# cure-lab/PnPInversion

Hardware: AMD Instinct MI355X
Metric: edited images/sec @ 512x512, 50 DDIM-inv + 50 denoise steps (higher is better)
Workload: dtype f16 (fp32 accumulate; latents / scheduler math fp32); 1 GPU; single 512x512 image per rank, SD-1.x (seeded synthetic weights), directinversion+p2p, faithful schedule: 650 UNet sample-forwards + 1 VAE encode + 5 VAE decodes per image, Refine+Reweight+LocalBlend controller; text K/V projected once per loop (not per forward); ddim_steps=50, schedule=lockstep

## Files before the change

### pnpinversion_amd/csrc/api.hip

```cpp
#include <math.h>
#include <stdio.h>
#include <stdlib.h>
#include <string.h>

#include <algorithm>
#include <functional>
#include <memory>
#include <string>

#include "model.h"

static int g_text_kv = 1;
static int g_temb_cache = 1;

static int fail(pnpi_ctx* c, int status, const char* what) {
  c->err = what;
  return status;
}
static int fail_launch(pnpi_ctx* c, int code, const char* what) {
  char buf[640];
  if (code > 0) {
    snprintf(buf, sizeof(buf), "HIP error %d (%s) in %s", code, hipGetErrorString((hipError_t)code), what);
    c->err = buf;
    return PNPI_EHIP;
// ... 201 lines not shown
  void* arena = nullptr;
  if (c->warena_ref && c->warena_ref->refs.fetch_sub(1) == 1) { arena = c->warena_ref->base; delete c->warena_ref; }
  void* bufs[] = {arena, c->persist.base, c->temp.base, c->ctrl_arena.base, c->splitk_ws, c->gn_partial, c->gn_bwd_ws,
                  c->temb_table, c->temb_h, c->temb_emb, c->bias_scratch, c->bias_tab, c->tkv.base, c->rows_ident};
  for (void* b : bufs) (void)hipFree(b);
  if (c->tape) {
    (void)hipFree(c->tape->garena.base); (void)hipFree(c->tape->d_ctx); (void)hipFree(c->tape->attn_scratch);
    for (auto& kv : c->tape->wd) (void)hipFree(kv.second);
    delete c->tape;
  }
  delete c;
}

static void invalidate_derived(pnpi_ctx* c) {
  std::fill(c->bias_valid.begin(), c->bias_valid.end(), 0);
  c->tkv.rows = 0; c->tkv.use = false;
  if (c->tape) { for (auto& kv : c->tape->wd) (void)hipFree(kv.second); c->tape->wd.clear(); }
}

int pnpi_load_weights(pnpi_ctx* c, const pnpi_named_tensor* ts, int n) {
  if (!c || !ts) return PNPI_EINVAL;
  if (c->warena_borrowed) return fail(c, PNPI_ESTATE, "this context borrows its weights (pnpi_create_shared): load them into the owning context");
  invalidate_derived(c);
  for (int i = 0; i < n; ++i) {
    const pnpi_named_tensor& t = ts[i];
    std::string name = t.name;
    size_t pos = name.find(".downsamplers.0.Conv2d_0.");
    if (pos != std::string::npos) name.replace(pos, strlen(".downsamplers.0.Conv2d_0."), ".downsamplers.0.conv.");
    if (name.compare(0, 16, "clip.text_model.") == 0) name = "clip." + name.substr(16);
    auto it = c->slots.find(name);
    if (it == c->slots.end()) continue;
    Slot& s = it->second;
    size_t numel = 1;
    for (int d = 0; d < t.ndim; ++d) numel *= (size_t)t.shape[d];
    if (s.kind == 0) {
      if (numel != (size_t)s.rows * s.cols * s.taps) { c->err = "shape mismatch for " + name; return PNPI_ESHAPE; }
      CK(launch_repack_matrix(t.data, t.dtype, s.rows, s.cols, s.taps, (half_t*)s.dst, s.dst_ld, s.cin_pad, s.row0, s.dh, s.Dp, c->st,
                              s.ilv_half));
    } else {
      if (numel != (size_t)s.n) { c->err = "shape mismatch for " + name; return PNPI_ESHAPE; }
      CK(launch_repack_vec(t.data, t.dtype, s.n, (float*)s.dst, c->st, s.ilv_half));
    }
    s.loaded = true;
  }
  return 0;
}

int pnpi_missing_weights(const pnpi_ctx* c, char* names_out, size_t cap) {
  int missing = 0;
  size_t used = 0;
  if (names_out && cap) names_out[0] = 0;
  for (auto& kv : c->slots)
    if (!kv.second.loaded && kv.first.compare(0, 5, "clip.") != 0) {
      ++missing;
      if (names_out && used + kv.first.size() + 2 < cap) {
        memcpy(names_out + used, kv.first.c_str(), kv.first.size());
        used += kv.first.size();
        names_out[used++] = '\n';
        names_out[used] = 0;
      }
    }
  return missing;
}

int pnpi_weight_arena(pnpi_ctx* c, void** ptr, size_t* bytes) {
  if (!c || !ptr || !bytes) return PNPI_EINVAL;
  *ptr = c->warena.base; *bytes = c->warena.cap;
  return 0;
}

int pnpi_mark_all_loaded(pnpi_ctx* c) {
  invalidate_derived(c);
  for (auto& kv : c->slots) kv.second.loaded = true;
  return 0;
}

int pnpi_set_scheduler(pnpi_ctx* c, const float* ac, int n_train, float final_alpha) {
  if (!c || !ac || n_train != c->cfg.n_train_timesteps) return PNPI_EINVAL;
  c->ac.assign(ac, ac + n_train);
  c->final_alpha = final_alpha;
  c->sched_set = true;
  return 0;
}

int pnpi_get_counters(const pnpi_ctx* c, pnpi_counters* out) { if (!c || !out) return PNPI_EINVAL; *out = c->ctr; return 0; }
int pnpi_reset_counters(pnpi_ctx* c) { if (!c) return PNPI_EINVAL; memset(&c->ctr, 0, sizeof(c->ctr)); return 0; }

__global__ void __launch_bounds__(512, 2) mfma_clock_kernel(int iters, float* sink) {
  const int lane = threadIdx.x & 63;
  unsigned h = (unsigned)(blockIdx.x * 512 + threadIdx.x) * 2654435761u;
  half8 a, b;
#pragma unroll
  for (int j = 0; j < 8; ++j) {
    h ^= h >> 16; h *= 0x85ebca6bu; h ^= h >> 13;
    a[j] = (half_t)((float)(h & 0xffff) * (2.f / 65536.f) - 1.f);
    b[j] = (half_t)((float)(h >> 16) * (2.f / 65536.f) - 1.f);
// ... 322 lines not shown
int pnpi_op_conv(pnpi_ctx* c, const void* x1, const void* x2, int C1, int C2, int B, int H, int W, int ksize, int stride, int pad,
                 int ups, int Ho, int Wo, const void* w, const float* bias, const void* res, int N, void* out, int force_cfg,
                 int force_split) {
  return conv_hook(c, x1, x2, C1, C2, B, H, W, ksize, stride, pad, ups, Ho, Wo, w, bias, res, N, out, force_cfg, force_split, nullptr, nullptr);
}
int pnpi_op_conv_stats(pnpi_ctx* c, const void* x1, const void* x2, int C1, int C2, int B, int H, int W, int ksize, int stride, int pad,
                       int ups, int Ho, int Wo, const void* w, const float* bias, const void* res, int N, void* out, int force_cfg,
                       int force_split, float* stats_out, int* tile_rows_out) {
  if (!c || !stats_out || !tile_rows_out) return PNPI_EINVAL;
  return conv_hook(c, x1, x2, C1, C2, B, H, W, ksize, stride, pad, ups, Ho, Wo, w, bias, res, N, out, force_cfg, force_split, stats_out, tile_rows_out);
}
int pnpi_tile_table_lookup(int M, int N, int K, int ksize, int* cfg, int* split, int* entry_m) {
  return igemm_table_lookup(M, N, K, ksize, cfg, split, entry_m);
}
int pnpi_set_tuning(const char* key, int value) {
  if (!key) return PNPI_EINVAL;
  if (!strcmp(key, "text_kv")) { g_text_kv = value; return 0; }
  if (!strcmp(key, "temb_cache")) { g_temb_cache = value; return 0; }
  if (!strcmp(key, "gn_inline_rows")) { norm_set_tuning_gn_inline_rows(value); return 0; }
  if (!strcmp(key, "attn_vt_perm")) { g_vt_perm = value; return 0; }
  if (!strcmp(key, "attn_aug")) { g_attn_aug = value; return 0; }
  if (!strcmp(key, "attn_pipe")) return attn_set_tuning_pipe(value) == 0 ? 0 : PNPI_EINVAL;
  if (!strcmp(key, "gn_slab")) { g_gn_slab = value; return 0; }
  if (!strcmp(key, "op_attention_aug")) { g_op_attention_aug = value; return 0; }
  if (!strcmp(key, "op_attention_vt_perm")) { g_op_attention_vt_perm = value; return 0; }
  if (!strcmp(key, "attn_bwd_flash")) { g_attn_bwd_flash = value; return 0; }
  return igemm_set_tuning(key, value) == 0 ? 0 : PNPI_EINVAL;
}
int pnpi_op_gemm(pnpi_ctx* c, const void* a, int lda, const void* w, int ldw, int M, int N, int K, float alpha, const float* bias,
                 const void* res, void* out, int ldo, int vt_col0, void* outT, int vt_ld, int vt_f32, int rpb, int force_cfg,
                 int force_split) {
  GemmP p; gemm_defaults(p);
  p.x1 = (const half_t*)a; p.C1 = K; p.ldx1 = lda; p.B = 1; p.H = 1; p.W = M; p.Ho = 1; p.Wo = M; p.ksize = 1;
  p.w = (const half_t*)w; p.ldw = ldw; p.M = M; p.N = N; p.K = K; p.alpha = alpha; p.bias = bias; p.res = (const half_t*)res;
  p.ldres = N; p.out = (half_t*)out; p.ldo = ldo;
  if (outT) { p.outT = outT; p.vt_col0 = vt_col0; p.vt_ld = vt_ld; p.vt_f32 = vt_f32; p.rows_per_batch = rpb; }
  CK(launch_igemm(p, c->splitk_ws, c->splitk_bytes, c->st, force_cfg, force_split));
  return 0;
}
int pnpi_op_gemm_geglu(pnpi_ctx* c, const void* a, int lda, const void* w, int ldw, int M, int N, int K, const float* bias, void* out,
                       int ldo) {
  GemmP p; gemm_defaults(p);
  p.x1 = (const half_t*)a; p.C1 = K; p.ldx1 = lda; p.B = 1; p.H = 1; p.W = M; p.Ho = 1; p.Wo = M; p.ksize = 1;
  p.w = (const half_t*)w; p.ldw = ldw; p.M = M; p.N = N; p.K = K; p.bias = bias; p.out = (half_t*)out; p.ldo = ldo; p.geglu = 1;
  CK(launch_igemm(p, c->splitk_ws, c->splitk_bytes, c->st));
  return 0;
// ... 112 lines not shown
```

### pnpinversion_amd/csrc/api_graph.inc

```
static void prof_open(pnpi_ctx* c, ProfRec& r) {
  (void)hipEventCreate(&r.a); (void)hipEventCreate(&r.b);
  (void)hipEventRecord(r.a, c->st);
}
static void prof_close(pnpi_ctx* c, ProfRec& r, int cls, double flops, double bytes, int M = 0, int N = 0, int K = 0, int ks = 0) {
  (void)hipEventRecord(r.b, c->st);
  r.cls = cls; r.flops = flops; r.bytes = bytes; r.M = M; r.N = N; r.K = K; r.ksize = ks;
  c->prof.push_back(r);
}
static int g_gn_slab = 0;
static int flush_pending(pnpi_ctx* c) {
  if (!c->pend_on) return 0;
  c->pend_on = false;
  return launch_splitk_reduce(c->pend, c->st);
}
#define PROF(cls, flops, bytes, expr) PROFD(cls, flops, bytes, 0, 0, 0, expr)
#define PROFD(cls, flops, bytes, d0, d1, d2, expr)            \
  do {                                                        \
    if (c->pend_on) { int _f = flush_pending(c); if (_f) return fail_launch(c, _f, "deferred split-K combine"); } \
    if (c->prof_on && !c->dry) {                              \
      ProfRec _pr; prof_open(c, _pr);                         \
      int _r = (expr);                                        \
      prof_close(c, _pr, (cls), (flops), (bytes), (d0), (d1), (d2)); \
      if (_r) return fail_launch(c, _r, #expr);               \
    } else {                                                  \
      int _r = (expr);                                        \
      if (_r) return fail_launch(c, _r, #expr);               \
    }                                                         \
  } while (0)

enum { TK_CONV = 0, TK_GEMM = 1, TK_GN = 2, TK_LN = 3, TK_ATTN = 4, TK_GEGLU = 5, TK_TRANSPOSE_V = 6 };
struct TapeOp {
  int kind = 0;
// ... 269 lines not shown
      int srow = cur_step < cd.n_alpha_rows ? cur_step : cd.n_alpha_rows - 1;
      e.c1 = cd.coef + ((size_t)srow * 2 + 0) * cd.npairs * 96;
      e.c2 = cd.coef + ((size_t)srow * 2 + 1) * cd.npairs * 96;
      const bool lb = cd.lb_any && t.lb_slot0 >= 0 && N == c->unet.lb_tokens;
      e.lb_alpha = lb ? cd.lb_alpha : nullptr;
      e.lb_acc = lb ? cd.lb_acc : nullptr;
      e.lb_slot0 = t.lb_slot0; e.lb_nslots = c->unet.lb_nslots; e.lb_planes = cd.lb_planes; e.write_src = 0;
      PROF(PNPI_KC_ATTN_EDIT, 4.0 * 2 * cd.npairs * t.heads * (double)N * T * t.dh, 0.0, launch_attn_cross_edit(e, c->st));
    }
  }
  half_t* hs2 = talloc(c, (size_t)M * C);
  CK(op_gemm(c, ao2, C, M, C, t.o2.w, C, C, t.o2.b, hs1, C, hs2, C));

  half_t* n3 = talloc(c, (size_t)M * C);
  if (!c->dry) PROF(PNPI_KC_LAYERNORM, 0.0, 2.0 * M * (double)C * 2.0, launch_layernorm(hs2, M, C, 1e-5f, t.ln3.g, t.ln3.b, n3, c->st));
  half_t* f2 = talloc(c, (size_t)M * 4 * C);
  if (C % 64 == 0) {
    CK(op_gemm(c, n3, C, M, C, t.ff1.w, C, 8 * C, t.ff1.b, nullptr, 0, f2, 4 * C, 1.f, nullptr, -1.0, 1));
  } else {
    half_t* f1 = talloc(c, (size_t)M * 8 * C);
    CK(op_gemm(c, n3, C, M, C, t.ff1.w, C, 8 * C, t.ff1.b, nullptr, 0, f1, 8 * C));
    if (!c->dry) PROF(PNPI_KC_GEGLU, 0.0, 12.0 * M * (double)C * 2.0, launch_geglu(f1, M, 4 * C, f2, c->st));
  }
  half_t* hs3 = talloc(c, (size_t)M * C);
  CK(op_gemm(c, f2, 4 * C, M, 4 * C, t.ff2.w, 4 * C, C, t.ff2.b, hs2, C, hs3, C));
  StatsReq qo;
  CK(op_conv(c, hs3, C, nullptr, 0, B, H, W, t.proj_out, 1, 0, 0, t.proj_out.b, x, out, H, W, -1, nullptr, &qo));
  if (so) { so->p = qo.buf; so->rows = qo.rows; }
  c->temp.release(mk);
  return 0;
}

static int op_ln(pnpi_ctx* c, const half_t* x, int M, int C, const NormW& nw, half_t* out) {
  if (c->dry) return 0;
  if (taping(c)) { TapeOp o; o.kind = TK_LN; o.x1 = x; o.M = M; o.C1 = C; o.nw = &nw; o.eps = 1e-5f; o.out = out; c->tape->ops.push_back(o); }
  PROF(PNPI_KC_LAYERNORM, 0.0, 2.0 * M * (double)C * 2.0, launch_layernorm(x, M, C, 1e-5f, nw.g, nw.b, out, c->st));
  return 0;
}
static int transformer_fwd_tape(pnpi_ctx* c, const TransformerW& t, const half_t* x, int B, int H, int W, const half_t* ctx16, half_t* out) {
  const pnpi_model_config& g = c->cfg;
  c->tf_index++;
  const int C = t.C, N = H * W, M = B * N, hd = t.heads * t.Dp, X = g.cross_dim, T = g.ctx_len;
  const float scale = 1.0f / sqrtf((float)t.dh);
  half_t* g0 = talloc(c, (size_t)M * C);
  CK(op_gn(c, x, nullptr, C, 0, B, N, t.gn, g.norm_groups, 1e-6f, 0, g0));
  half_t* hs = talloc(c, (size_t)M * C);
  CK(op_conv(c, g0, C, nullptr, 0, B, H, W, t.proj_in, 1, 0, 0, t.proj_in.b, nullptr, hs, H, W));
  half_t* n1 = talloc(c, (size_t)M * C);
  CK(op_ln(c, hs, M, C, t.ln1, n1));
  half_t* qkv = talloc(c, (size_t)M * 3 * hd);
// ... 332 lines not shown
```

### pnpinversion_amd/csrc/api_weights.inc

```
static void reg_mat(pnpi_ctx* c, const std::string& name, half_t* dst, int rows, int cols, int taps, int dst_ld, int cin_pad,
                    int row0 = 0, int dh = 0, int Dp = 0) {
  Slot s; s.kind = 0; s.dst = dst; s.rows = rows; s.cols = cols; s.taps = taps; s.dst_ld = dst_ld; s.cin_pad = cin_pad;
  s.row0 = row0; s.dh = dh; s.Dp = Dp; s.n = 0; s.ilv_half = 0; s.loaded = false;
  c->slots[name] = s;
}
static void reg_vec(pnpi_ctx* c, const std::string& name, float* dst, int n) {
  Slot s; s.kind = 1; s.dst = dst; s.rows = 0; s.cols = 0; s.taps = 0; s.dst_ld = 0; s.cin_pad = 0; s.row0 = 0; s.dh = 0; s.Dp = 0;
  s.n = n; s.ilv_half = 0; s.loaded = false;
  c->slots[name] = s;
}
static half_t* walloc_h(pnpi_ctx* c, size_t n) { return (half_t*)c->warena.alloc(n * sizeof(half_t)); }
static float* walloc_f(pnpi_ctx* c, size_t n) { return (float*)c->warena.alloc(n * sizeof(float)); }

static ConvW make_conv(pnpi_ctx* c, const std::string& pre, int cin, int cout, int k, int cout_alloc = 0, float* bias_dst = nullptr) {
  ConvW w; w.cin = cin; w.cin_pad = round_up_i(cin, 8); w.cout = cout; w.k = k;
  int ra = cout_alloc > cout ? cout_alloc : cout;
  w.w = walloc_h(c, (size_t)ra * k * k * w.cin_pad);
  w.b = bias_dst ? bias_dst : walloc_f(c, ra);
  reg_mat(c, pre + ".weight", w.w, cout, cin, k * k, k * k * w.cin_pad, w.cin_pad);
  reg_vec(c, pre + ".bias", w.b, cout);
  return w;
}
static LinW make_lin(pnpi_ctx* c, const std::string& pre, int in, int out) {
  LinW l; l.in = in; l.out = out;
// ... 40 lines not shown
  t.ln2 = make_norm(c, tb + ".norm2", C);
  t.ln3 = make_norm(c, tb + ".norm3", C);
  t.w_qkv = walloc_h(c, (size_t)3 * hd * C);
  reg_mat(c, tb + ".attn1.to_q.weight", t.w_qkv, C, C, 1, C, C, 0, t.dh, t.Dp);
  reg_mat(c, tb + ".attn1.to_k.weight", t.w_qkv, C, C, 1, C, C, hd, t.dh, t.Dp);
  reg_mat(c, tb + ".attn1.to_v.weight", t.w_qkv, C, C, 1, C, C, 2 * hd, t.dh, t.Dp);
  t.b_qkv_aug = nullptr;
  if (t.Dp == 64 && t.dh == 40) {
    t.b_qkv_aug = walloc_f(c, (size_t)3 * hd);
    c->aug_biases.push_back({t.b_qkv_aug, t.heads, t.Dp, t.dh});
  }
  t.o1 = make_lin(c, tb + ".attn1.to_out.0", C, C);
  t.w_q2 = walloc_h(c, (size_t)hd * C);
  reg_mat(c, tb + ".attn2.to_q.weight", t.w_q2, C, C, 1, C, C, 0, t.dh, t.Dp);
  t.w_kv2 = walloc_h(c, (size_t)2 * hd * X);
  reg_mat(c, tb + ".attn2.to_k.weight", t.w_kv2, C, X, 1, X, X, 0, t.dh, t.Dp);
  reg_mat(c, tb + ".attn2.to_v.weight", t.w_kv2, C, X, 1, X, X, hd, t.dh, t.Dp);
  t.o2 = make_lin(c, tb + ".attn2.to_out.0", C, C);
  t.ff1 = make_lin(c, tb + ".ff.net.0.proj", C, 8 * C);
  c->slots[tb + ".ff.net.0.proj.weight"].ilv_half = 4 * C;
  c->slots[tb + ".ff.net.0.proj.bias"].ilv_half = 4 * C;
  t.ff2 = make_lin(c, tb + ".ff.net.2", 4 * C, C);
  t.proj_out = make_conv(c, pre + ".proj_out", C, C, 1);
  return t;
}
static VaeAttnW make_vae_attn(pnpi_ctx* c, const std::string& pre, int C) {
  VaeAttnW a; a.C = C;
  a.gn = make_norm(c, pre + ".group_norm", C);
  a.w_qkv = walloc_h(c, (size_t)3 * C * C);
  a.b_qkv = walloc_f(c, 3 * C);
  reg_mat(c, pre + ".query.weight", a.w_qkv, C, C, 1, C, C, 0);
  reg_mat(c, pre + ".key.weight", a.w_qkv, C, C, 1, C, C, C);
  reg_mat(c, pre + ".value.weight", a.w_qkv, C, C, 1, C, C, 2 * C);
  reg_vec(c, pre + ".query.bias", a.b_qkv, C);
  reg_vec(c, pre + ".key.bias", a.b_qkv + C, C);
  reg_vec(c, pre + ".value.bias", a.b_qkv + 2 * C, C);
  a.proj = make_lin(c, pre + ".proj_attn", C, C);
  return a;
}

static int temb_total_channels(const pnpi_model_config& g) {
  int n = g.n_blocks, total = 0;
  for (int i = 0; i < n; ++i) total += g.layers_per_block * g.block_out_channels[i];
  total += 2 * g.block_out_channels[n - 1];
  for (int i = 0; i < n; ++i) total += (g.layers_per_block + 1) * g.block_out_channels[n - 1 - i];
  return total;
}

static void build_model(pnpi_ctx* c) {
  const pnpi_model_config& g = c->cfg;
  c->slots.clear();
  c->aug_biases.clear();
  UNetW& u = c->unet;
  u = UNetW();
  const int n = g.n_blocks, C0 = g.block_out_channels[0], TE = 4 * C0;
  const int sumC = temb_total_channels(g);
  u.temb_w = walloc_h(c, (size_t)sumC * TE);
  u.temb_b = walloc_f(c, sumC);
  u.conv1_b = walloc_f(c, sumC);
  u.temb_total = 0;
  u.conv_in = make_conv(c, "unet.conv_in", g.in_channels, C0, 3);
  u.t1 = make_lin(c, "unet.time_embedding.linear_1", C0, TE);
  u.t2 = make_lin(c, "unet.time_embedding.linear_2", TE, TE);
  std::vector<TransformerW*> down_stored, up_stored;
  int out_ch = C0;
  u.down_res.resize(n); u.down_attn.resize(n);
  for (int i = 0; i < n; ++i) {
    int in_ch = out_ch; out_ch = g.block_out_channels[i];
    for (int j = 0; j < g.layers_per_block; ++j) {
      std::string pre = "unet.down_blocks." + std::to_string(i);
      u.down_res[i].push_back(make_resnet(c, pre + ".resnets." + std::to_string(j), j == 0 ? in_ch : out_ch, out_ch, true));
      if (g.block_has_attn[i]) u.down_attn[i].push_back(make_transformer(c, pre + ".attentions." + std::to_string(j), out_ch, 0));
    }
    if (i != n - 1) u.down_samp.push_back(make_conv(c, "unet.down_blocks." + std::to_string(i) + ".downsamplers.0.conv", out_ch, out_ch, 3));
  }
// ... 110 lines not shown
```

### pnpinversion_amd/csrc/model.h

```cpp
#pragma once
#include <atomic>
#include <string>
#include <unordered_map>
#include <vector>

#include "../../include/pnpi.h"
#include "ops.h"

static inline size_t align_up(size_t x, size_t a) { return (x + a - 1) / a * a; }
static inline int round_up_i(int x, int a) { return (x + a - 1) / a * a; }

struct Bump {
  char* base = nullptr;
  size_t cap = 0, off = 0, peak = 0;
  bool overflow = false;
  void* alloc(size_t bytes) {
    off = align_up(off, 256);
    size_t at = off;
    off += bytes;
    if (off > peak) peak = off;
    if (base && off > cap) { overflow = true; return base; }
    return base ? (void*)(base + at) : (void*)(uintptr_t)(0x1000 + at);
  }
  size_t mark() const { return off; }
// ... 14 lines not shown
struct LinW { half_t* w; float* b; int in, out; };
struct NormW { float* g; float* b; int c; };

struct ResnetW {
  NormW n1, n2;
  ConvW c1, c2, sc;
  bool has_sc;
  int temb_off;
  int cin, cout;
};

struct TransformerW {
  int C, heads, dh, Dp;
  NormW gn, ln1, ln2, ln3;
  ConvW proj_in, proj_out;
  half_t* w_qkv;
  float* b_qkv_aug;
  LinW o1;
  half_t* w_q2;
  half_t* w_kv2;
  LinW o2;
  LinW ff1;
  LinW ff2;
  int place;
  int lb_slot0;
};

struct VaeAttnW {
  int C;
  NormW gn;
  half_t* w_qkv; float* b_qkv;
  LinW proj;
};

struct UNetW {
  ConvW conv_in, conv_out;
  NormW norm_out;
  LinW t1, t2;
  half_t* temb_w;
  float* temb_b;
  float* conv1_b;
  int temb_total;
  std::vector<std::vector<ResnetW>> down_res;
  std::vector<std::vector<TransformerW>> down_attn;
  std::vector<ConvW> down_samp;
  ResnetW mid_res[2];
// ... 67 lines not shown

struct TextKV {
  std::vector<half_t*> k, vt;
  char* base = nullptr; size_t cap = 0;
  int rows = 0;
  bool use = false;
};

struct ProfRec { int cls; double flops, bytes; hipEvent_t a, b; int M, N, K, ksize; int cfg = -1, split = 0; int geom[7] = {0, 0, 0, 0, 0, 0, 0}; };

struct Tape;

struct pnpi_ctx {
  pnpi_model_config cfg;
  int device;
  hipStream_t st;
  std::string err;
  int max_rows, max_vae;
  bool dry;
  int tf_index = 0;
  Bump warena, persist, temp, ctrl_arena;
  struct AugBias { float* p; int heads, Dp, dh; };
  std::vector<AugBias> aug_biases;
  bool warena_borrowed = false;
  struct ArenaRef { void* base; std::atomic<int> refs; };
  ArenaRef* warena_ref = nullptr;
  float* splitk_ws; size_t splitk_bytes;
  float* gn_partial;
  float* temb_table;
  float* temb_h;
  float* temb_emb;
  float* bias_eff;
  float* bias_scratch;
  float* bias_tab = nullptr;
  std::vector<char> bias_valid;
  TextKV tkv;
  pnpi_attn_callback attn_cb = nullptr;
  float* gn_bwd_ws = nullptr; size_t gn_bwd_ws_floats = 0;
  void* attn_cb_user = nullptr;
  float* attn_buf = nullptr; size_t attn_buf_bytes = 0;
  std::unordered_map<std::string, Slot> slots;
  UNetW unet;
  VaeW vae;
  ClipW clip;
  int* rows_ident = nullptr;
  int rows_ident_n = 0;
  std::vector<float> ac;
  float final_alpha;
// ... 10 lines not shown
```

### pnpinversion_amd/csrc/norm.hip

```cpp
#include <algorithm>
#include "ops.h"

__global__ void __launch_bounds__(256) gn_stats_kernel(const half_t* __restrict__ x1, const half_t* __restrict__ x2, int C1,
                                                       int C2, int HW, int G, int nchunk, float* __restrict__ partial) {
  extern __shared__ __attribute__((aligned(16))) char smem_raw[];
  float* s_part = reinterpret_cast<float*>(smem_raw);
  const int C = C1 + C2, C8 = C >> 3;
  const int b = blockIdx.x, chunk = blockIdx.y;
  const int TC = C8 < 256 ? C8 : 256;
  const int TP = 256 / TC;
  const int tc = threadIdx.x % TC, tp = threadIdx.x / TC;
  const int ppc = (HW + nchunk - 1) / nchunk;
  const int p0 = chunk * ppc, p1 = min(HW, p0 + ppc);
  if (tp < TP) {
    for (int cv = tc; cv < C8; cv += TC) {
      float s[8], q[8];
#pragma unroll
      for (int j = 0; j < 8; ++j) { s[j] = 0.f; q[j] = 0.f; }
      const int c = cv * 8;
      const half_t* src; int ld, cc;
      if (c < C1) { src = x1; ld = C1; cc = c; } else { src = x2; ld = C2; cc = c - C1; }
      const half_t* base = src + (size_t)b * HW * ld + cc;
      int pix = p0 + tp;
      for (; pix + 3 * TP < p1; pix += 4 * TP) {
// ... 756 lines not shown
  }
}
int launch_repack_matrix(const void* src, int src_f16, int rows, int cols, int taps, half_t* dst, int dst_ld, int cin_pad, int row0,
                         int dh, int Dp, hipStream_t st, int ilv_half) {
  size_t total = (size_t)rows * cols * taps;
  int blocks = (int)((total + 255) / 256);
  if (blocks > 4096) blocks = 4096;
  if (blocks < 1) blocks = 1;
  repack_matrix_kernel<<<blocks, 256, 0, st>>>(src, src_f16, rows, cols, taps, dst, dst_ld, cin_pad, row0, dh, Dp, ilv_half);
  return (int)hipGetLastError();
}
__global__ void repack_vec_kernel(const void* __restrict__ src, int src_f16, int n, float* __restrict__ dst, int ilv_half) {
  for (int i = blockIdx.x * blockDim.x + threadIdx.x; i < n; i += gridDim.x * blockDim.x)
    dst[ilv_row(i, ilv_half)] = src_f16 ? (float)((const half_t*)src)[i] : ((const float*)src)[i];
}
int launch_repack_vec(const void* src, int src_f16, int n, float* dst, hipStream_t st, int ilv_half) {
  int blocks = (n + 255) / 256;
  if (blocks > 1024) blocks = 1024;
  if (blocks < 1) blocks = 1;
  repack_vec_kernel<<<blocks, 256, 0, st>>>(src, src_f16, n, dst, ilv_half);
  return (int)hipGetLastError();
}


__global__ void embed_tokens_kernel(const int* __restrict__ ids, int M, int T, int H, int vocab, const half_t* __restrict__ tok,
                                    const half_t* __restrict__ pos, half_t* __restrict__ out) {
  const size_t total = (size_t)M * H;
  for (size_t i = (size_t)blockIdx.x * blockDim.x + threadIdx.x; i < total; i += (size_t)gridDim.x * blockDim.x) {
    const int m = (int)(i / H), c = (int)(i - (size_t)m * H);
    int id = ids[m];
    id = id < 0 ? 0 : (id >= vocab ? vocab - 1 : id);
    out[i] = (half_t)((float)tok[(size_t)id * H + c] + (float)pos[(size_t)(m % T) * H + c]);
  }
}
int launch_embed_tokens(const int* ids, int M, int T, int H, int vocab, const half_t* tok_emb, const half_t* pos_emb, half_t* out,
                        hipStream_t st) {
  const size_t total = (size_t)M * H;
  int blocks = (int)((total + 255) / 256); if (blocks > 2048) blocks = 2048; if (blocks < 1) blocks = 1;
  embed_tokens_kernel<<<blocks, 256, 0, st>>>(ids, M, T, H, vocab, tok_emb, pos_emb, out);
  return (int)hipGetLastError();
}
__global__ void quick_gelu_kernel(half_t* __restrict__ x, size_t n) {
  for (size_t i = (size_t)blockIdx.x * blockDim.x + threadIdx.x; i < n; i += (size_t)gridDim.x * blockDim.x) {
    const float v = (float)x[i];
    x[i] = (half_t)(v / (1.f + __expf(-1.702f * v)));
  }
// ... 15 lines not shown
```

### pnpinversion_amd/csrc/ops.h

```cpp
#pragma once
#include "common.h"

struct GemmP {
  const half_t* x1; const half_t* x2;
  int C1, C2, ldx1, ldx2;
  int B, H, W, Ho, Wo;
  int ksize, stride, pad, ups;
  const half_t* w; int ldw;
  int M, N, K;
  const float* bias;
  const half_t* res; int ldres;
  float alpha;
  half_t* out; int ldo;
  void* outT; int vt_col0, vt_ld, vt_f32, rows_per_batch;
  int vt_perm16;
  float* slab; int splitk, kchunks_per_split;
  float* stats;
  int geglu;
  int epi_lds;
  int bias_init;
  int res_late;
  int k_order;
  int gx, gy, gz, tile_order;
  int nbatch;
// ... 10 lines not shown
void igemm_set_dma(int on);

int launch_groupnorm(const half_t* x1, const half_t* x2, int C1, int C2, int B, int HW, int G, float eps,
                     const float* gamma, const float* beta, int silu, half_t* out, float* partial, hipStream_t st);
int launch_groupnorm_fused(const half_t* x1, const half_t* x2, int C1, int C2, int B, int HW, int G, float eps,
                           const float* gamma, const float* beta, int silu, half_t* out, const float* st1, int tpb1,
                           const float* st2, int tpb2, float* scratch, hipStream_t st);
void norm_set_tuning_gn_inline_rows(int v);
struct GnSlab { const float* slab; int splitk; size_t stride; const float* bias; const half_t* res; int ldres; half_t* sum_out; };
bool groupnorm_slab_ok(int C1, int C2, int HW, int G);
int launch_groupnorm_slab(const GnSlab& sl, const half_t* x2, int C1, int C2, int B, int HW, int G, float eps, const float* gamma,
                          const float* beta, int silu, half_t* out, hipStream_t st);
int launch_layernorm(const half_t* x, int M, int C, float eps, const float* gamma, const float* beta, half_t* out,
                     hipStream_t st);
int launch_geglu(const half_t* x, int M, int I, half_t* out, hipStream_t st);
int launch_softmax_rows(half_t* x, int M, int N, int ld, hipStream_t st);
int launch_softmax_rows_f32(float* x, size_t M, int N, hipStream_t st);
int launch_f32_rows_to_f16_padded(const float* in, size_t M, int N, int ld, half_t* out, hipStream_t st);
int launch_gemv(const float* x, int K, const half_t* W, int N, const float* bias, const float* bias2, int silu_in,
                float* out, hipStream_t st);
int launch_repack_matrix(const void* src, int src_f16, int rows, int cols, int taps, half_t* dst, int dst_ld, int cin_pad,
                         int row0, int dh, int Dp, hipStream_t st, int ilv_half = 0);
int launch_repack_vec(const void* src, int src_f16, int n, float* dst, hipStream_t st, int ilv_half = 0);
int launch_nchw_f32_to_nhwc_f16(const float* in, int B, int C, int HW, int Cp, half_t* out, hipStream_t st);
int launch_f32_to_f16(const float* in, size_t n, half_t* out, hipStream_t st);
int launch_img_u8_to_nhwc(const uint8_t* img, int n, int HW, int Cp, half_t* out, hipStream_t st);
int launch_dec_to_u8(const float* nchw, int n, int HW, uint8_t* out_hwc, hipStream_t st);
int launch_scale_f32(const float* in, size_t n, float s, float* out, hipStream_t st);
int launch_gather_rows_f32(const float* in, const int* rows, int nrows, size_t row_elems, float* out, hipStream_t st);
int launch_embed_tokens(const int* ids, int M, int T, int H, int vocab, const half_t* tok_emb, const half_t* pos_emb, half_t* out,
                        hipStream_t st);
int launch_quick_gelu(half_t* x, size_t n, hipStream_t st);
int launch_f16_to_f32(const half_t* in, size_t n, float* out, hipStream_t st);

__host__ __device__ inline int vt_perm16_pos(int tok) { return tok ^ ((((tok >> 2) ^ (tok >> 3)) & 1) ? 12 : 0); }

struct AttnP {
  const half_t* q; int ldq, q_off;
  const half_t* k; int ldk, k_off;
  const half_t* vt; int ldv;
  half_t* o; int ldo;
  int heads, Nq, Nk, Dp, dh;
  float scale;
  const int* rows;
  int nrows;
  int causal = 0;
// ... 94 lines not shown
```

### pnpinversion_amd/csrc/tile_table.inc

```
{64, 1280, 1280, 1, 1, 4},
{64, 1280, 2560, 1, 1, 12},
{64, 1280, 3840, 1, 1, 12},
{64, 1280, 5120, 1, 11, 12},
{64, 1280, 10240, 1, 1, 12},
{64, 1280, 11520, 3, 1, 12},
{64, 1280, 23040, 3, 1, 12},
{64, 2560, 1280, 1, 11, 4},
{64, 2560, 11520, 3, 1, 6},
{64, 3840, 1280, 1, 1, 1},
{64, 5120, 1280, 1, 1, 3},
{64, 10240, 1280, 1, 1, 1},
{77, 768, 1024, 1, 11, 8},
{77, 768, 1536, 1, 1, 8},
{77, 768, 2560, 1, 1, 8},
{77, 1024, 768, 1, 1, 4},
{77, 1536, 768, 1, 1, 4},
{77, 2560, 768, 1, 1, 1},
{192, 1280, 1280, 1, 1, 4},
{192, 1280, 2560, 1, 11, 4},
{192, 1280, 5120, 1, 1, 8},
{192, 1280, 11520, 3, 1, 8},
{192, 1280, 23040, 3, 11, 8},
{192, 3840, 1280, 1, 1, 1},
{192, 10240, 1280, 1, 1, 1},
{256, 640, 1280, 1, 11, 4},
{256, 640, 5760, 3, 1, 12},
{256, 640, 11520, 3, 1, 12},
{256, 1280, 640, 1, 8, 1},
{256, 1280, 1280, 1, 11, 3},
{256, 1280, 1920, 1, 11, 3},
{256, 1280, 2560, 1, 1, 3},
{256, 1280, 3840, 1, 1, 3},
{256, 1280, 5120, 1, 1, 6},
{256, 1280, 5760, 3, 1, 6},
{256, 1280, 10240, 1, 1, 6},
{256, 1280, 11520, 3, 14, 12},
{256, 1280, 17280, 3, 14, 12},
{256, 1280, 23040, 3, 0, 12},
{256, 1920, 1280, 1, 8, 1},
{256, 1920, 11520, 3, 0, 8},
{256, 2560, 1280, 1, 8, 1},
{256, 2560, 11520, 3, 14, 12},
{256, 3840, 1280, 1, 8, 1},
{256, 5120, 1280, 1, 1, 1},
{256, 10240, 1280, 1, 18, 1},
{512, 1280, 1280, 1, 8, 1},
{512, 1280, 2560, 1, 8, 1},
{512, 1280, 5120, 1, 11, 3},
{512, 1280, 11520, 3, 14, 12},
{512, 1280, 23040, 3, 16, 16},
{512, 3840, 1280, 1, 11, 1},
{512, 10240, 1280, 1, 1, 1},
{768, 640, 5760, 3, 11, 4},
{768, 1280, 640, 1, 8, 1},
{768, 1280, 1280, 1, 8, 1},
{768, 1280, 1920, 1, 8, 1},
{768, 1280, 2560, 1, 8, 1},
{768, 1280, 5120, 1, 18, 4},
{768, 1280, 5760, 3, 18, 4},
{768, 1280, 11520, 3, 18, 4},
{768, 1280, 17280, 3, 16, 16},
{768, 1280, 23040, 3, 16, 16},
{768, 3840, 1280, 1, 18, 1},
{768, 10240, 1280, 1, 14, 1},
{1024, 320, 640, 1, 1, 1},
{1024, 320, 2880, 3, 1, 6},
{1024, 320, 5760, 3, 11, 4},
{1024, 640, 320, 1, 8, 1},
{1024, 640, 640, 1, 8, 1},
{1024, 640, 768, 1, 8, 1},
{1024, 640, 960, 1, 8, 1},
{1024, 640, 1280, 1, 8, 1},
{1024, 640, 1920, 1, 8, 1},
{1024, 640, 2304, 1, 11, 3},
{1024, 640, 2560, 1, 11, 3},
{1024, 640, 2880, 3, 1, 3},
{1024, 640, 5120, 1, 11, 3},
{1024, 640, 5760, 3, 11, 3},
{1024, 640, 8640, 3, 14, 12},
{1024, 640, 11520, 3, 14, 12},
{1024, 640, 17280, 3, 14, 12},
{1024, 768, 640, 1, 8, 1},
{1024, 960, 640, 1, 1, 1},
{1024, 960, 5760, 3, 11, 2},
{1024, 1280, 640, 1, 11, 1},
{1024, 1280, 1280, 1, 11, 1},
{1024, 1280, 1920, 1, 11, 1},
{1024, 1280, 2560, 1, 11, 1},
{1024, 1280, 5120, 1, 14, 6},
{1024, 1280, 5760, 3, 14, 6},
{1024, 1280, 11520, 3, 16, 12},
{1024, 1280, 17280, 3, 16, 12},
{1024, 1280, 23040, 3, 16, 12},
{1024, 1920, 640, 1, 1, 1},
{1024, 1920, 5760, 3, 16, 8},
{1024, 2304, 640, 1, 1, 1},
{1024, 2560, 640, 1, 1, 1},
{1024, 3840, 1280, 1, 10, 1},
{1024, 5120, 640, 1, 14, 1},
// ... 9 lines not shown
{2048, 1280, 17280, 3, 16, 6},
{2048, 1280, 23040, 3, 16, 6},
{2048, 3840, 1280, 1, 14, 1},
{2048, 10240, 1280, 1, 0, 1},
{3072, 320, 2880, 3, 11, 2},
{3072, 640, 320, 1, 11, 1},
{3072, 640, 640, 1, 11, 1},
{3072, 640, 960, 1, 11, 1},
{3072, 640, 1280, 1, 11, 1},
{3072, 640, 1920, 1, 11, 1},
{3072, 640, 2560, 1, 11, 1},
{3072, 640, 2880, 3, 11, 1},
{3072, 640, 5760, 3, 18, 2},
{3072, 640, 8640, 3, 17, 8},
{3072, 640, 11520, 3, 17, 8},
{3072, 640, 17280, 3, 17, 8},
{3072, 768, 640, 1, 1, 1},
{3072, 1280, 640, 1, 18, 1},
{3072, 1280, 1280, 1, 18, 1},
{3072, 1280, 1920, 1, 18, 1},
{3072, 1280, 2560, 1, 18, 1},
{3072, 1280, 5120, 1, 16, 4},
{3072, 1280, 5760, 3, 16, 4},
{3072, 1280, 11520, 3, 16, 4},
{3072, 1280, 17280, 3, 16, 4},
{3072, 1280, 23040, 3, 16, 4},
{3072, 2304, 640, 1, 14, 1},
{3072, 3840, 1280, 1, 17, 1},
{3072, 5120, 640, 1, 17, 1},
{3072, 10240, 1280, 1, 17, 1},
{4096, 4, 8, 1, 1, 1},
{4096, 4, 2880, 3, 11, 4},
{4096, 8, 8, 1, 1, 1},
{4096, 8, 4608, 3, 1, 12},
{4096, 320, 72, 3, 1, 1},
{4096, 320, 320, 1, 1, 1},
{4096, 320, 512, 1, 1, 1},
{4096, 320, 640, 1, 11, 1},
{4096, 320, 960, 1, 1, 1},
{4096, 320, 1280, 1, 1, 1},
{4096, 320, 1536, 1, 1, 1},
{4096, 320, 2560, 1, 1, 1},
{4096, 320, 2880, 3, 11, 1},
{4096, 320, 5760, 3, 11, 3},
{4096, 320, 8640, 3, 17, 8},
{4096, 512, 72, 3, 1, 1},
{4096, 512, 320, 1, 1, 1},
{4096, 512, 512, 1, 1, 1},
{4096, 512, 4096, 1, 11, 1},
{4096, 512, 4608, 3, 11, 1},
{4096, 640, 320, 1, 1, 1},
{4096, 640, 640, 1, 1, 1},
{4096, 640, 960, 1, 1, 1},
{4096, 640, 1280, 1, 1, 1},
{4096, 640, 1920, 1, 1, 1},
{4096, 640, 2560, 1, 1, 1},
{4096, 640, 2880, 3, 1, 1},
{4096, 640, 5760, 3, 14, 3},
{4096, 640, 8640, 3, 17, 4},
{4096, 640, 11520, 3, 17, 4},
{4096, 640, 17280, 3, 17, 4},
{4096, 768, 640, 1, 1, 1},
{4096, 960, 320, 1, 10, 1},
{4096, 960, 2880, 3, 10, 1},
// ... 32 lines not shown
{8192, 640, 17280, 3, 17, 2},
{8192, 768, 640, 1, 14, 1},
{8192, 1280, 11520, 3, 16, 3},
{8192, 1536, 512, 1, 16, 1},
{8192, 2304, 640, 1, 14, 1},
{8192, 5120, 640, 1, 17, 1},
{12288, 4, 2880, 3, 1, 4},
{12288, 320, 72, 3, 1, 1},
{12288, 320, 320, 1, 14, 1},
{12288, 320, 640, 1, 14, 1},
{12288, 320, 960, 1, 14, 1},
{12288, 320, 1280, 1, 11, 1},
{12288, 320, 2880, 3, 11, 1},
{12288, 320, 5760, 3, 17, 4},
{12288, 320, 8640, 3, 17, 4},
{12288, 512, 320, 1, 14, 1},
{12288, 640, 320, 1, 14, 1},
{12288, 640, 640, 1, 14, 1},
{12288, 640, 960, 1, 14, 1},
{12288, 640, 1280, 1, 14, 1},
{12288, 640, 1920, 1, 14, 1},
{12288, 640, 2560, 1, 14, 1},
{12288, 640, 2880, 3, 14, 1},
{12288, 640, 5760, 3, 17, 2},
{12288, 640, 8640, 3, 17, 2},
{12288, 640, 11520, 3, 17, 2},
{12288, 640, 17280, 3, 17, 2},
{12288, 768, 640, 1, 17, 1},
{12288, 1280, 11520, 3, 16, 1},
{12288, 1536, 320, 1, 14, 1},
{12288, 2304, 640, 1, 16, 1},
{12288, 2560, 320, 1, 17, 1},
{12288, 5120, 640, 1, 17, 1},
{16384, 4, 2880, 3, 8, 1},
{16384, 256, 2304, 3, 10, 1},
{16384, 320, 72, 3, 1, 1},
{16384, 320, 320, 1, 14, 1},
{16384, 320, 640, 1, 0, 1},
{16384, 320, 960, 1, 14, 1},
{16384, 320, 1280, 1, 14, 1},
{16384, 320, 2880, 3, 14, 1},
{16384, 320, 5760, 3, 17, 2},
{16384, 320, 8640, 3, 17, 2},
{16384, 512, 256, 1, 14, 1},
{16384, 512, 320, 1, 14, 1},
{16384, 512, 2304, 3, 14, 1},
// ... 16 lines not shown
{32768, 4, 2880, 3, 11, 1},
{32768, 256, 2304, 3, 14, 1},
{32768, 320, 72, 3, 1, 1},
{32768, 320, 320, 1, 0, 1},
{32768, 320, 640, 1, 17, 1},
{32768, 320, 960, 1, 17, 1},
{32768, 320, 1280, 1, 17, 1},
{32768, 320, 2880, 3, 17, 1},
{32768, 320, 5760, 3, 17, 1},
{32768, 320, 8640, 3, 17, 1},
{32768, 512, 256, 1, 16, 1},
{32768, 512, 320, 1, 16, 1},
{32768, 512, 2304, 3, 16, 1},
{32768, 512, 4608, 3, 16, 1},
{32768, 640, 5760, 3, 17, 1},
{32768, 1536, 320, 1, 16, 1},
{32768, 2560, 320, 1, 0, 1},
{49152, 4, 2880, 3, 1, 1},
{49152, 320, 72, 3, 1, 1},
{49152, 320, 320, 1, 17, 1},
{49152, 320, 640, 1, 17, 1},
{49152, 320, 960, 1, 17, 1},
{49152, 320, 1280, 1, 17, 1},
{49152, 320, 2880, 3, 17, 1},
{49152, 320, 5760, 3, 17, 1},
{49152, 320, 8640, 3, 17, 1},
{49152, 512, 320, 1, 17, 1},
{49152, 640, 5760, 3, 17, 1},
{49152, 1536, 320, 1, 16, 1},
{49152, 2560, 320, 1, 0, 1},
{65536, 128, 1152, 3, 14, 1},
{65536, 256, 128, 1, 16, 1},
{65536, 256, 512, 1, 16, 1},
{65536, 256, 1152, 3, 16, 1},
{65536, 256, 2304, 3, 16, 1},
{65536, 256, 4608, 3, 16, 1},
{65536, 512, 4608, 3, 16, 1},
{98304, 320, 2880, 3, 17, 1},
{98304, 640, 320, 1, 17, 1},
{98304, 640, 640, 1, 17, 1},
{98304, 640, 960, 1, 17, 1},
{98304, 640, 1280, 1, 17, 1},
{98304, 640, 1920, 1, 17, 1},
{98304, 640, 2560, 1, 17, 1},
{98304, 640, 2880, 3, 17, 1},
{98304, 640, 5760, 3, 17, 1},
// ... 40 lines not shown
```

Before: 1.016 images/s.

## Fold FF2 linear into transformer proj_out as single concatenated-K GEMM

Precomputes a combined weight [Wp·W2 | Wp] and bias Wp·b2+bp at weight-load time so the feed-forward output projection and the block's proj_out 1x1 conv run as one GEMM over the concatenated GEGLU output and residual. This removes one GEMM launch and the round trip of the intermediate hs3 activation. It adds a small fold kernel at load, extra weight memory, tile-table entries for the new K=5C shapes, and f16 rounding of the pre-multiplied weight.

```diff
diff --git a/pnpinversion_amd/csrc/api.hip b/pnpinversion_amd/csrc/api.hip
--- a/pnpinversion_amd/csrc/api.hip
+++ b/pnpinversion_amd/csrc/api.hip
@@ -247,6 +247,7 @@
   if (!c || !ts) return PNPI_EINVAL;
   if (c->warena_borrowed) return fail(c, PNPI_ESTATE, "this context borrows its weights (pnpi_create_shared): load them into the owning context");
   invalidate_derived(c);
+  bool fold_src = false;
   for (int i = 0; i < n; ++i) {
     const pnpi_named_tensor& t = ts[i];
     std::string name = t.name;
@@ -267,7 +268,9 @@
       CK(launch_repack_vec(t.data, t.dtype, s.n, (float*)s.dst, c->st, s.ilv_half));
     }
     s.loaded = true;
-  }
+    if (!fold_src && ff_fold_source(c, name)) { fold_src = true; c->warena_ref->ff_fold_ready = false; }
+  }
+  if (fold_src) CK(build_ff_fold(c));
   return 0;
 }
 
@@ -297,6 +300,7 @@
 int pnpi_mark_all_loaded(pnpi_ctx* c) {
   invalidate_derived(c);
   for (auto& kv : c->slots) kv.second.loaded = true;
+  CK(build_ff_fold(c));
   return 0;
 }
 
@@ -665,6 +669,7 @@
   if (!strcmp(key, "attn_aug")) { g_attn_aug = value; return 0; }
   if (!strcmp(key, "attn_pipe")) return attn_set_tuning_pipe(value) == 0 ? 0 : PNPI_EINVAL;
   if (!strcmp(key, "gn_slab")) { g_gn_slab = value; return 0; }
+  if (!strcmp(key, "ff_fold")) { g_ff_fold = value; return 0; }
   if (!strcmp(key, "op_attention_aug")) { g_op_attention_aug = value; return 0; }
   if (!strcmp(key, "op_attention_vt_perm")) { g_op_attention_vt_perm = value; return 0; }
   if (!strcmp(key, "attn_bwd_flash")) { g_attn_bwd_flash = value; return 0; }
diff --git a/pnpinversion_amd/csrc/api_graph.inc b/pnpinversion_amd/csrc/api_graph.inc
--- a/pnpinversion_amd/csrc/api_graph.inc
+++ b/pnpinversion_amd/csrc/api_graph.inc
@@ -8,6 +8,7 @@
   c->prof.push_back(r);
 }
 static int g_gn_slab = 0;
+static int g_ff_fold = 1;
 static int flush_pending(pnpi_ctx* c) {
   if (!c->pend_on) return 0;
   c->pend_on = false;
@@ -323,10 +324,15 @@
     CK(op_gemm(c, n3, C, M, C, t.ff1.w, C, 8 * C, t.ff1.b, nullptr, 0, f1, 8 * C));
     if (!c->dry) PROF(PNPI_KC_GEGLU, 0.0, 12.0 * M * (double)C * 2.0, launch_geglu(f1, M, 4 * C, f2, c->st));
   }
-  half_t* hs3 = talloc(c, (size_t)M * C);
-  CK(op_gemm(c, f2, 4 * C, M, 4 * C, t.ff2.w, 4 * C, C, t.ff2.b, hs2, C, hs3, C));
   StatsReq qo;
-  CK(op_conv(c, hs3, C, nullptr, 0, B, H, W, t.proj_out, 1, 0, 0, t.proj_out.b, x, out, H, W, -1, nullptr, &qo));
+  const bool fold = g_ff_fold && !c->dry && C % 64 == 0 && t.fo.w && c->warena_ref && c->warena_ref->ff_fold_ready && !keep_acts(c);
+  if (fold) {
+    CK(op_conv(c, f2, 4 * C, hs2, C, B, H, W, t.fo, 1, 0, 0, t.fo.b, x, out, H, W, -1, nullptr, &qo));
+  } else {
+    half_t* hs3 = talloc(c, (size_t)M * C);
+    CK(op_gemm(c, f2, 4 * C, M, 4 * C, t.ff2.w, 4 * C, C, t.ff2.b, hs2, C, hs3, C));
+    CK(op_conv(c, hs3, C, nullptr, 0, B, H, W, t.proj_out, 1, 0, 0, t.proj_out.b, x, out, H, W, -1, nullptr, &qo));
+  }
   if (so) { so->p = qo.buf; so->rows = qo.rows; }
   c->temp.release(mk);
   return 0;
diff --git a/pnpinversion_amd/csrc/api_weights.inc b/pnpinversion_amd/csrc/api_weights.inc
--- a/pnpinversion_amd/csrc/api_weights.inc
+++ b/pnpinversion_amd/csrc/api_weights.inc
@@ -86,6 +86,13 @@
   c->slots[tb + ".ff.net.0.proj.bias"].ilv_half = 4 * C;
   t.ff2 = make_lin(c, tb + ".ff.net.2", 4 * C, C);
   t.proj_out = make_conv(c, pre + ".proj_out", C, C, 1);
+  t.fo = ConvW{nullptr, nullptr, 5 * C, 5 * C, C, 1};
+  if (C % 64 == 0) {
+    t.fo.w = walloc_h(c, (size_t)C * 5 * C);
+    t.fo.b = walloc_f(c, C);
+    c->ff_folds.push_back({t.proj_out.w, t.proj_out.cin_pad, t.proj_out.b, t.ff2.w, t.ff2.b, C, t.fo.w, t.fo.b,
+                           {pre + ".proj_out.weight", pre + ".proj_out.bias", tb + ".ff.net.2.weight", tb + ".ff.net.2.bias"}});
+  }
   return t;
 }
 static VaeAttnW make_vae_attn(pnpi_ctx* c, const std::string& pre, int C) {
@@ -103,6 +110,26 @@
   return a;
 }
 
+static bool ff_fold_source(const pnpi_ctx* c, const std::string& name) {
+  for (const pnpi_ctx::FfFold& f : c->ff_folds)
+    for (const std::string& s : f.src) if (s == name) return true;
+  return false;
+}
+static int build_ff_fold(pnpi_ctx* c) {
+  if (c->warena_borrowed || !c->warena_ref) return 0;
+  c->warena_ref->ff_fold_ready = false;
+  if (c->ff_folds.empty()) return 0;
+  for (const pnpi_ctx::FfFold& f : c->ff_folds)
+    for (const std::string& s : f.src) {
+      auto it = c->slots.find(s);
+      if (it == c->slots.end() || !it->second.loaded) return 0;
+    }
+  for (const pnpi_ctx::FfFold& f : c->ff_folds)
+    if (int r = launch_ff_fold_weights(f.wp, f.ldp, f.bp, f.w2, f.b2, f.C, f.w_fo, f.b_fo, c->st)) return r;
+  c->warena_ref->ff_fold_ready = true;
+  return 0;
+}
+
 static int temb_total_channels(const pnpi_model_config& g) {
   int n = g.n_blocks, total = 0;
   for (int i = 0; i < n; ++i) total += g.layers_per_block * g.block_out_channels[i];
@@ -115,6 +142,7 @@
   const pnpi_model_config& g = c->cfg;
   c->slots.clear();
   c->aug_biases.clear();
+  c->ff_folds.clear();
   UNetW& u = c->unet;
   u = UNetW();
   const int n = g.n_blocks, C0 = g.block_out_channels[0], TE = 4 * C0;
diff --git a/pnpinversion_amd/csrc/model.h b/pnpinversion_amd/csrc/model.h
--- a/pnpinversion_amd/csrc/model.h
+++ b/pnpinversion_amd/csrc/model.h
@@ -60,6 +60,7 @@
   LinW o2;
   LinW ff1;
   LinW ff2;
+  ConvW fo;
   int place;
   int lb_slot0;
 };
@@ -173,8 +174,10 @@
   Bump warena, persist, temp, ctrl_arena;
   struct AugBias { float* p; int heads, Dp, dh; };
   std::vector<AugBias> aug_biases;
+  struct FfFold { const half_t* wp; int ldp; const float* bp; const half_t* w2; const float* b2; int C; half_t* w_fo; float* b_fo; std::string src[4]; };
+  std::vector<FfFold> ff_folds;
   bool warena_borrowed = false;
-  struct ArenaRef { void* base; std::atomic<int> refs; };
+  struct ArenaRef { void* base; std::atomic<int> refs; bool ff_fold_ready = false; };
   ArenaRef* warena_ref = nullptr;
   float* splitk_ws; size_t splitk_bytes;
   float* gn_partial;
diff --git a/pnpinversion_amd/csrc/norm.hip b/pnpinversion_amd/csrc/norm.hip
--- a/pnpinversion_amd/csrc/norm.hip
+++ b/pnpinversion_amd/csrc/norm.hip
@@ -802,6 +802,65 @@
   return (int)hipGetLastError();
 }
 
+__global__ void __launch_bounds__(256) ff_fold_weight_kernel(const half_t* __restrict__ wp, int ldp, const half_t* __restrict__ w2, int C,
+                                                             half_t* __restrict__ w_fo) {
+  const int tid = threadIdx.x, n0 = blockIdx.y * 64, k0 = blockIdx.x * 64, K4 = 4 * C, ldo = 5 * C;
+  if (k0 >= K4) {
+    for (int idx = tid; idx < 64 * 16; idx += 256) {
+      const int r = idx >> 4, v = (idx & 15) * 4;
+      *reinterpret_cast<half4*>(w_fo + (size_t)(n0 + r) * ldo + k0 + v) = *reinterpret_cast<const half4*>(wp + (size_t)(n0 + r) * ldp + (k0 - K4) + v);
+    }
+    return;
+  }
+  __shared__ float sA[16][64 + 4];
+  __shared__ float sB[16][64 + 4];
+  const int tx = tid & 15, ty = tid >> 4;
+  float acc[4][4];
+#pragma unroll
+  for (int a = 0; a < 4; ++a)
+#pragma unroll
+    for (int b = 0; b < 4; ++b) acc[a][b] = 0.f;
+  for (int j0 = 0; j0 < C; j0 += 16) {
+    const half4 av = *reinterpret_cast<const half4*>(wp + (size_t)(n0 + (tid >> 2)) * ldp + j0 + (tid & 3) * 4);
+    const half4 bv = *reinterpret_cast<const half4*>(w2 + (size_t)(j0 + ty) * K4 + k0 + tx * 4);
+#pragma unroll
+    for (int q = 0; q < 4; ++q) { sA[(tid & 3) * 4 + q][tid >> 2] = (float)av[q]; sB[ty][tx * 4 + q] = (float)bv[q]; }
+    __syncthreads();
+#pragma unroll
+    for (int jj = 0; jj < 16; ++jj) {
+      float a4[4], b4[4];
+#pragma unroll
+      for (int q = 0; q < 4; ++q) { a4[q] = sA[jj][ty * 4 + q]; b4[q] = sB[jj][tx * 4 + q]; }
+#pragma unroll
+      for (int a = 0; a < 4; ++a)
+#pragma unroll
+        for (int b = 0; b < 4; ++b) acc[a][b] = __builtin_fmaf(a4[a], b4[b], acc[a][b]);
+    }
+    __syncthreads();
+  }
+#pragma unroll
+  for (int a = 0; a < 4; ++a) {
+    const half4 h = {(half_t)acc[a][0], (half_t)acc[a][1], (half_t)acc[a][2], (half_t)acc[a][3]};
+    *reinterpret_cast<half4*>(w_fo + (size_t)(n0 + ty * 4 + a) * ldo + k0 + tx * 4) = h;
+  }
+}
+__global__ void __launch_bounds__(256) ff_fold_bias_kernel(const half_t* __restrict__ wp, int ldp, const float* __restrict__ b2,
+                                                           const float* __restrict__ bp, int C, float* __restrict__ b_fo) {
+  const int n = blockIdx.x * 4 + (threadIdx.x >> 6), lane = threadIdx.x & 63;
+  if (n >= C) return;
+  float s = 0.f;
+  for (int j = lane; j < C; j += 64) s = __builtin_fmaf((float)wp[(size_t)n * ldp + j], b2[j], s);
+  s = wave_sum(s);
+  if (lane == 0) b_fo[n] = s + bp[n];
+}
+int launch_ff_fold_weights(const half_t* wp, int ldp, const float* bp, const half_t* w2, const float* b2, int C, half_t* w_fo, float* b_fo,
+                           hipStream_t st) {
+  if (C <= 0 || C % 64 || ldp < C || ldp % 4) return -2;
+  ff_fold_weight_kernel<<<dim3(5 * C / 64, C / 64), 256, 0, st>>>(wp, ldp, w2, C, w_fo);
+  ff_fold_bias_kernel<<<(C + 3) / 4, 256, 0, st>>>(wp, ldp, b2, bp, C, b_fo);
+  return (int)hipGetLastError();
+}
+
 
 __global__ void embed_tokens_kernel(const int* __restrict__ ids, int M, int T, int H, int vocab, const half_t* __restrict__ tok,
                                     const half_t* __restrict__ pos, half_t* __restrict__ out) {
diff --git a/pnpinversion_amd/csrc/ops.h b/pnpinversion_amd/csrc/ops.h
--- a/pnpinversion_amd/csrc/ops.h
+++ b/pnpinversion_amd/csrc/ops.h
@@ -56,6 +56,8 @@
 int launch_repack_matrix(const void* src, int src_f16, int rows, int cols, int taps, half_t* dst, int dst_ld, int cin_pad,
                          int row0, int dh, int Dp, hipStream_t st, int ilv_half = 0);
 int launch_repack_vec(const void* src, int src_f16, int n, float* dst, hipStream_t st, int ilv_half = 0);
+int launch_ff_fold_weights(const half_t* wp, int ldp, const float* bp, const half_t* w2, const float* b2, int C, half_t* w_fo, float* b_fo,
+                           hipStream_t st);
 int launch_nchw_f32_to_nhwc_f16(const float* in, int B, int C, int HW, int Cp, half_t* out, hipStream_t st);
 int launch_f32_to_f16(const float* in, size_t n, half_t* out, hipStream_t st);
 int launch_img_u8_to_nhwc(const uint8_t* img, int n, int HW, int Cp, half_t* out, hipStream_t st);
diff --git a/pnpinversion_amd/csrc/tile_table.inc b/pnpinversion_amd/csrc/tile_table.inc
--- a/pnpinversion_amd/csrc/tile_table.inc
+++ b/pnpinversion_amd/csrc/tile_table.inc
@@ -2,6 +2,7 @@
 {64, 1280, 2560, 1, 1, 12},
 {64, 1280, 3840, 1, 1, 12},
 {64, 1280, 5120, 1, 11, 12},
+{64, 1280, 6400, 1, 1, 12},
 {64, 1280, 10240, 1, 1, 12},
 {64, 1280, 11520, 3, 1, 12},
 {64, 1280, 23040, 3, 1, 12},
@@ -33,6 +34,7 @@
 {256, 1280, 3840, 1, 1, 3},
 {256, 1280, 5120, 1, 1, 6},
 {256, 1280, 5760, 3, 1, 6},
+{256, 1280, 6400, 1, 18, 12},
 {256, 1280, 10240, 1, 1, 6},
 {256, 1280, 11520, 3, 14, 12},
 {256, 1280, 17280, 3, 14, 12},
@@ -58,6 +60,7 @@
 {768, 1280, 2560, 1, 8, 1},
 {768, 1280, 5120, 1, 18, 4},
 {768, 1280, 5760, 3, 18, 4},
+{768, 1280, 6400, 1, 18, 4},
 {768, 1280, 11520, 3, 18, 4},
 {768, 1280, 17280, 3, 16, 16},
 {768, 1280, 23040, 3, 16, 16},
@@ -75,6 +78,7 @@
 {1024, 640, 2304, 1, 11, 3},
 {1024, 640, 2560, 1, 11, 3},
 {1024, 640, 2880, 3, 1, 3},
+{1024, 640, 3200, 1, 11, 3},
 {1024, 640, 5120, 1, 11, 3},
 {1024, 640, 5760, 3, 11, 3},
 {1024, 640, 8640, 3, 14, 12},
@@ -130,6 +134,7 @@
 {3072, 1280, 2560, 1, 18, 1},
 {3072, 1280, 5120, 1, 16, 4},
 {3072, 1280, 5760, 3, 16, 4},
+{3072, 1280, 6400, 1, 16, 4},
 {3072, 1280, 11520, 3, 16, 4},
 {3072, 1280, 17280, 3, 16, 4},
 {3072, 1280, 23040, 3, 16, 4},
@@ -148,6 +153,7 @@
 {4096, 320, 960, 1, 1, 1},
 {4096, 320, 1280, 1, 1, 1},
 {4096, 320, 1536, 1, 1, 1},
+{4096, 320, 1600, 1, 11, 1},
 {4096, 320, 2560, 1, 1, 1},
 {4096, 320, 2880, 3, 11, 1},
 {4096, 320, 5760, 3, 11, 3},
@@ -226,6 +232,7 @@
 {12288, 640, 1920, 1, 14, 1},
 {12288, 640, 2560, 1, 14, 1},
 {12288, 640, 2880, 3, 14, 1},
+{12288, 640, 3200, 1, 14, 1},
 {12288, 640, 5760, 3, 17, 2},
 {12288, 640, 8640, 3, 17, 2},
 {12288, 640, 11520, 3, 17, 2},
@@ -288,6 +295,7 @@
 {49152, 320, 640, 1, 17, 1},
 {49152, 320, 960, 1, 17, 1},
 {49152, 320, 1280, 1, 17, 1},
+{49152, 320, 1600, 1, 17, 1},
 {49152, 320, 2880, 3, 17, 1},
 {49152, 320, 5760, 3, 17, 1},
 {49152, 320, 8640, 3, 17, 1},
```

Measured after the change: 1.034 images/s (median of 6 runs). +1.7%, better.
